# Chang-Tun-Yu/HLS-final-Visual-Odometry

Measured on AMD Instinct MI355X. Metric: stereo frame-pairs/sec (detect+match), KITTI 1241x376; matches bit-exact, higher is better.
Workload: dtype u8; 1 GPU; KITTI 1241x376 stereo quad-match (prev/curr x L/R), default 50x50 bins; noise=0, gpu_max_hw_queues=4, streams_per_gpu=256, frames_in_hbm=8, parallelism=1x independent stream groups

## Files before the change

hls-final-visual-odometry_amd/csrc/kernels_detect.hip:

```cpp
#include "vh_dev.h"
#include <type_traits>

namespace {

__global__ void half_res_kernel(VhImages src, uint8_t *__restrict__ dst, VhGeom g) {
  const int32_t id = blockIdx.z;
  const uint8_t *__restrict__ I = vh_image_ptr(src, id);
  uint8_t *__restrict__ O = dst + (int64_t)id * g.bplm * g.Hm;
  const int32_t u = blockIdx.x * blockDim.x + threadIdx.x;
  const int32_t v = blockIdx.y;
  if (u >= g.bplm) return;
  uint32_t val = 0;
  if (u < g.Wm) {
    const int64_t r0 = (int64_t)(2 * v) * g.bpl + 2 * u, r1 = r0 + g.bpl;
    val = ((uint32_t)I[r0] + I[r0 + 1] + I[r1] + I[r1 + 1]) >> 2;
  }
  O[(int64_t)v * g.bplm + u] = (uint8_t)val;
}

__global__ void __launch_bounds__(256)
detect_nms_kernel(VhImages im, VhGeom g, uint64_t *__restrict__ rec, int32_t *__restrict__ chunk_count) {
  extern __shared__ __attribute__((aligned(16))) uint8_t smem[];
  uint8_t *sI = smem;
  int16_t *sF1 = (int16_t *)(smem + (size_t)g.IH * g.IWp);
  int16_t *sF2 = sF1 + (size_t)g.FH * g.FWp;

  const int32_t id = blockIdx.z;
  const uint8_t *__restrict__ I = vh_image_ptr(im, id);
  const int32_t n = g.n, n1 = n + 1;
  const int32_t bx0 = blockIdx.x * g.tbx, by0 = blockIdx.y * g.tby;
  const int32_t fx0 = VH_MARGIN + bx0 * n1, fy0 = VH_MARGIN + by0 * n1;
  const int32_t ix0 = fx0 - 2, iy0 = fy0 - 2;
  const int32_t tid = threadIdx.x;

  for (int32_t k = tid; k < g.IH * g.IWp; k += 256) {
    const int32_t r = k / g.IWp, c = k - r * g.IWp;
    const int32_t gx = ix0 + c, gy = iy0 + r;
    uint8_t v = 0;
    if (c < g.IW && gx < g.bplm && gy < g.Hm) v = I[(int64_t)gy * g.bplm + gx];
    sI[k] = v;
  }
  __syncthreads();

  {
    const int32_t nseg = max(1, 256 / g.FW);
    const int32_t rows_per = (g.FH + nseg - 1) / nseg;
    for (int32_t task = tid; task < g.FW * nseg; task += 256) {
      const int32_t seg = task / g.FW, cx = task - seg * g.FW;
      const int32_t r0 = seg * rows_per, r1 = min(g.FH, r0 + rows_per);
      if (r0 >= r1) continue;
      int32_t h5[5], h3[5], hc[5], cc[5];
#pragma unroll
      for (int32_t k = 0; k < 4; k++) {
        const uint8_t *p = sI + (size_t)(r0 + k) * g.IWp + cx;
        const int32_t a = p[0], b = p[1], c = p[2], d = p[3], e = p[4];
        h5[k + 1] = a + b + c + d + e; h3[k + 1] = b + c + d; hc[k + 1] = a + b - d - e; cc[k + 1] = c;
      }
      for (int32_t fr = r0; fr < r1; fr++) {
#pragma unroll
        for (int32_t k = 0; k < 4; k++) { h5[k] = h5[k + 1]; h3[k] = h3[k + 1]; hc[k] = hc[k + 1]; cc[k] = cc[k + 1]; }
        const uint8_t *p = sI + (size_t)(fr + 4) * g.IWp + cx;
        const int32_t a = p[0], b = p[1], c = p[2], d = p[3], e = p[4];
        h5[4] = a + b + c + d + e; h3[4] = b + c + d; hc[4] = a + b - d - e; cc[4] = c;
        const int32_t f2 = hc[0] + hc[1] - hc[3] - hc[4];
        const int32_t f1 = -(h5[0] + h5[1] + h5[2] + h5[3] + h5[4]) + 2 * (h3[1] + h3[2] + h3[3]) + 7 * cc[2];
        sF1[(size_t)fr * g.FWp + cx] = (int16_t)f1;
        sF2[(size_t)fr * g.FWp + cx] = (int16_t)f2;
      }
    }
  }
  __syncthreads();

  int32_t *sCnt = (int32_t *)(sF2 + (size_t)g.FH * g.FWp);
  uint32_t *sWork = (uint32_t *)(sCnt + 1);
  uint16_t *sCode = (uint16_t *)(sWork + 4 * g.tbx * g.tby);
  const int32_t nblk_tile = g.tbx * g.tby;
  if (tid == 0) *sCnt = 0;
  for (int32_t k = tid; k < 4 * nblk_tile; k += 256) sCode[k] = VH_NO_CODE;
  __syncthreads();
  const int32_t xlim = (g.Wm - 1 - VH_MARGIN) - fx0, ylim = (g.Hm - 1 - VH_MARGIN) - fy0;
  const int32_t lby = tid / g.tbx, lbx = tid - lby * g.tbx;
  const int32_t bx = bx0 + lbx, by = by0 + lby;
  const bool have_block = tid < nblk_tile && bx < g.nbx && by < g.nby;
  if (have_block) {
    const int32_t fx = n + lbx * n1, fy = n + lby * n1;
    int32_t ex[4], ey[4], ev[4];
    ex[0] = ex[1] = ex[2] = ex[3] = fx;
    ey[0] = ey[1] = ey[2] = ey[3] = fy;
    ev[0] = ev[1] = sF1[(size_t)fy * g.FWp + fx];
    ev[2] = ev[3] = sF2[(size_t)fy * g.FWp + fx];
    for (int32_t j2 = fy; j2 <= fy + n; j2++) {
      for (int32_t i2 = fx; i2 <= fx + n; i2++) {
        int32_t cur = sF1[(size_t)j2 * g.FWp + i2];
        if (cur < ev[0]) { ex[0] = i2; ey[0] = j2; ev[0] = cur; }
        else if (cur > ev[1]) { ex[1] = i2; ey[1] = j2; ev[1] = cur; }
        cur = sF2[(size_t)j2 * g.FWp + i2];
        if (cur < ev[2]) { ex[2] = i2; ey[2] = j2; ev[2] = cur; }
        else if (cur > ev[3]) { ex[3] = i2; ey[3] = j2; ev[3] = cur; }
      }
    }
#pragma unroll
    for (int32_t c = 0; c < 4; c++) {
      const bool pass = (c & 1) ? (ev[c] >= g.tau) : (ev[c] <= -g.tau);
      if (pass) sWork[atomicAdd(sCnt, 1)] = (uint32_t)ex[c] | ((uint32_t)ey[c] << 10) | ((uint32_t)c << 20) | ((uint32_t)tid << 22);
    }
  }
  __syncthreads();
  const int32_t nwork = *sCnt;
  for (int32_t w = tid; w < nwork; w += 256) {
    const uint32_t e = sWork[w];
    const int32_t cx = e & 1023, cy = (e >> 10) & 1023, c = (e >> 20) & 3, owner = e >> 22;
    const int32_t oby = owner / g.tbx, obx = owner - oby * g.tbx;
    const int32_t fx = n + obx * n1, fy = n + oby * n1;
    const int16_t *F = (c < 2) ? sF1 : sF2;
    const bool is_min = (c & 1) == 0;
    const int32_t val = F[(size_t)cy * g.FWp + cx];
    const int32_t jhi = min(cy + n, ylim), ihi = min(cx + n, xlim);
    bool ok = true;
    for (int32_t j2 = cy - n; j2 <= jhi && ok; j2++) {
      for (int32_t i2 = cx - n; i2 <= ihi; i2++) {
        const int32_t cur = F[(size_t)j2 * g.FWp + i2];
        const bool outside = (i2 < fx) | (i2 > fx + n) | (j2 < fy) | (j2 > fy + n);
        if (outside && (is_min ? (cur < val) : (cur > val))) { ok = false; break; }
      }
    }
    if (ok) sCode[owner * 4 + c] = (uint16_t)(((cy - fy) << 6) | (cx - fx));
  }
  __syncthreads();
  if (have_block) {
    uint64_t code = 0;
    int32_t cnt = 0;
#pragma unroll
    for (int32_t c = 0; c < 4; c++) {
      const uint32_t pc = sCode[tid * 4 + c];
      code |= (uint64_t)pc << (16 * c);
      cnt += pc != VH_NO_CODE ? 1 : 0;
    }
    const int32_t blk = by * g.nbx + bx;
    rec[(int64_t)id * g.nblocks + blk] = code;
    if (cnt) atomicAdd(&chunk_count[(int64_t)id * g.nchunks + blk / VH_CHUNK], cnt);
  }
}

#ifdef VH_EMIT_TIMING
__device__ unsigned long long g_emit_t[8];
extern "C" int32_t vh_debug_emit_timing(unsigned long long *out, int32_t reset) {
  if (hipMemcpyFromSymbol(out, HIP_SYMBOL(g_emit_t), sizeof(g_emit_t)) != hipSuccess) return -3;
  if (reset) { unsigned long long z[8] = {0}; z[6] = ~0ull; if (hipMemcpyToSymbol(HIP_SYMBOL(g_emit_t), z, sizeof(z)) != hipSuccess) return -3; }
  return 0;
}
#define VH_TICK_IMPL(k) do { __syncthreads(); if (t_on_) { const unsigned long long now_ = __builtin_readcyclecounter(); atomicAdd(&g_emit_t[k], now_ - t_prev_); t_prev_ = now_; if ((k) == 4) atomicMax(&g_emit_t[7], now_); } } while (0)
#define VH_TICK_INIT_IMPL const bool t_on_ = threadIdx.x == 0 && (blockIdx.x + gridDim.x * (blockIdx.y + gridDim.y * blockIdx.z)) % 61 == 0; unsigned long long t_prev_ = __builtin_readcyclecounter(); if (t_on_) { atomicAdd(&g_emit_t[5], 1ull); atomicMin(&g_emit_t[6], t_prev_); }
#endif
#if defined(VH_EMIT_TIMING) && VH_EMIT_TIMING == 2
#define VH_DTICK(k) VH_TICK_IMPL(k)
#define VH_DTICK_INIT VH_TICK_INIT_IMPL
#else
#define VH_DTICK(k) do { } while (0)
#define VH_DTICK_INIT do { } while (0)
#endif
#if defined(VH_EMIT_TIMING) && VH_EMIT_TIMING != 2
#define VH_ETICK(k) VH_TICK_IMPL(k)
#define VH_ETICK_INIT VH_TICK_INIT_IMPL
#else
#define VH_ETICK(k) do { } while (0)
#define VH_ETICK_INIT do { } while (0)
#endif

template <int N> struct DetTile {
  static constexpr int N1 = N + 1, TBX = 32, TBY = 8;
  static constexpr int FW = TBX * N1 + 2 * N, FH = TBY * N1 + 2 * N;
  static constexpr int IW = FW + 4, IH = FH + 4;
  static constexpr int OFF = (VH_MARGIN - 2) & 3;
  static constexpr int DW = (IW + 3 + 3) / 4;
  static constexpr int IP = DW * 4;
  static constexpr int groups(int px) { return (FW + OFF + px - 1) / px; }
  static constexpr int seg_cost(int px, int s) {
    const int rows = (FH + s - 1) / s, waves = (groups(px) * s + 63) / 64;
    const int hrow = px == 4 ? 28 : 18, vrow = px == 4 ? 26 : 13;
    return groups(px) * s > 256 || rows * (s - 1) >= FH ? (1 << 30) : 1000 * ((rows + 4) * hrow + rows * vrow) + waves;
  }
  static constexpr int best_seg(int px) {
    int b = 1;
    for (int s = 2; s <= 16; s++)
      if (seg_cost(px, s) < seg_cost(px, b)) b = s;
    return b;
  }
#ifdef VH_DET_PX
  static constexpr int PX = VH_DET_PX;
  static constexpr int SEG = VH_DET_SEG;
#else
  static constexpr int PX = seg_cost(2, best_seg(2)) < seg_cost(4, best_seg(4)) ? 2 : 4;
  static constexpr int SEG = best_seg(PX);
#endif
  static constexpr int G = groups(PX);
  static constexpr int FP = PX * G;
  static constexpr int ROWS = (FH + SEG - 1) / SEG;
  static constexpr int BIAS = 8192;
  static_assert((G - 1) * PX / 4 + 1 <= DW - 1, "a group reads the staged dword it starts in and the next one");
  static_assert(G * SEG <= 256, "one lane per (group, row segment)");
  static constexpr int LAST = FH - (SEG - 1) * ROWS;
  static_assert(LAST >= 1, "every segment has rows");
};

template <int N>
__global__ void __launch_bounds__(256)
detect_nms_fast_kernel(VhImages im, VhGeom g, uint64_t *__restrict__ rec, int32_t *__restrict__ chunk_count) {
  using T = DetTile<N>;
  constexpr int N1 = T::N1, WN = 2 * N + 1;
  VH_DET_SETPRIO();
  constexpr int X_BYTES = (T::IH * T::IP > 6144) ? T::IH * T::IP : 6144;
  __shared__ __attribute__((aligned(16))) int16_t sF1[T::FH * T::FP];
  __shared__ __attribute__((aligned(16))) int16_t sF2[T::FH * T::FP];
  __shared__ __attribute__((aligned(16))) uint8_t sX[X_BYTES];
  uint8_t *sI = sX;

  const int32_t id = blockIdx.z, tid = threadIdx.x;
  const uint8_t *__restrict__ I = vh_image_ptr(im, id);
  const int32_t bx0 = blockIdx.x * T::TBX, by0 = blockIdx.y * T::TBY;
  const int32_t fx0 = VH_MARGIN + bx0 * N1, fy0 = VH_MARGIN + by0 * N1;
  const int32_t ix0 = fx0 - 2, iy0 = fy0 - 2;
  const int32_t ax0 = ix0 - T::OFF;
  VH_DTICK_INIT;

  {
    constexpr int NLD = (T::IH * T::DW + 255) / 256;
    uint32_t stg[NLD];
    bool inside[NLD];
#pragma unroll
    for (int32_t i = 0; i < NLD; i++) {
      const int32_t k = min(tid + 256 * i, T::IH * T::DW - 1);
      const int32_t r = k / T::DW, c = k - r * T::DW;
      const int32_t gy = iy0 + r, gx = ax0 + 4 * c;
      stg[i] = *(const uint32_t *)(I + (int64_t)min(gy, g.Hm - 1) * g.bplm + min(gx, g.bplm - 4));
      inside[i] = gy < g.Hm && gx < g.bplm;
    }
    __builtin_amdgcn_sched_barrier(0);
#pragma unroll
    for (int32_t i = 0; i < NLD; i++) {
      const int32_t k = tid + 256 * i;
      if (k < T::IH * T::DW) ((uint32_t *)sI)[k] = inside[i] ? stg[i] : 0u;
    }
  }
  __syncthreads();

  VH_DTICK(0);
  if (tid < T::G * T::SEG) {
    constexpr int PX = T::PX, NR = PX / 2;
    const int32_t seg = tid / T::G, gq = tid - seg * T::G;
    const int32_t r0 = seg * T::ROWS;
    {
      constexpr uint32_t HB = 512u * 0x00010001u, KB = (uint32_t)T::BIAS * 0x00010001u;
      const uint32_t *p = (const uint32_t *)sI + r0 * T::DW + (gq * PX) / 4;
      const uint32_t sel0 = 0x0c010c00u + ((PX == 2 && (gq & 1)) ? 0x00020002u : 0u);
      uint32_t *o1 = (uint32_t *)sF1 + (r0 * T::FP + PX * gq) / 2, *o2 = (uint32_t *)sF2 + (r0 * T::FP + PX * gq) / 2;
      uint32_t h5[NR][5], h3[NR][5], pc[NR][4], cc[NR][5], hcp[NR], S5[NR];
#pragma unroll
      for (int32_t h = 0; h < NR; h++) S5[h] = 0u;
#pragma unroll
      for (int32_t t = 0; t < T::ROWS + 4; t++) {
        if (t - 4 < T::LAST || r0 + t - 4 < T::FH) {
          const uint32_t A = p[t * T::DW], B = p[t * T::DW + 1];
          uint32_t pk[PX + 3];
#pragma unroll
          for (int32_t k = 0; k < PX + 3; k++) pk[k] = __builtin_amdgcn_perm(B, A, sel0 + (uint32_t)k * 0x00010001u);
          uint32_t n5[NR], n3[NR], nc[NR], nz[NR];
          if (PX == 4) {
            const uint32_t a01 = pk[0] + pk[1], a23 = pk[2] + pk[3], a34 = pk[3] + pk[4], a56 = pk[5] + pk[6];
            n3[0] = a23 + pk[1];             n3[NR - 1] = a34 + pk[5];
            n5[0] = n3[0] + pk[0] + pk[4];   n5[NR - 1] = n3[NR - 1] + pk[2] + pk[6];
            nc[0] = (a01 + HB) - a34;        nc[NR - 1] = (a23 + HB) - a56;
            nz[0] = pk[2];                   nz[NR - 1] = pk[4];
          } else {
            n3[0] = pk[1] + pk[2] + pk[3];
            n5[0] = n3[0] + pk[0] + pk[4];
            nc[0] = ((pk[0] + pk[1]) + HB) - (pk[3] + pk[4]);
            nz[0] = pk[2];
          }
          uint32_t f1[NR], f2[NR];
#pragma unroll
          for (int32_t h = 0; h < NR; h++) {
            const uint32_t old5 = h5[h][0];
#pragma unroll
            for (int32_t k = 0; k < 4; k++) { h5[h][k] = h5[h][k + 1]; h3[h][k] = h3[h][k + 1]; cc[h][k] = cc[h][k + 1]; }
            h5[h][4] = n5[h]; h3[h][4] = n3[h]; cc[h][4] = nz[h];
            S5[h] += n5[h];
            if (t >= 5) S5[h] -= old5;
#pragma unroll
            for (int32_t k = 0; k < 3; k++) pc[h][k] = pc[h][k + 1];
            if (t > 0) pc[h][3] = hcp[h] + nc[h];
            hcp[h] = nc[h];
            if (t >= 4) {
              const uint32_t S3 = h3[h][1] + h3[h][2] + h3[h][3];
              f2[h] = (pc[h][0] + KB) - pc[h][3];
              f1[h] = ((S3 + S3) + (__umul24(cc[h][2], 7u) + KB)) - S5[h];
            }
          }
          if (t >= 4) {
            if (PX == 4) {
              *(uint2 *)(o1 + (t - 4) * (T::FP / 2)) = make_uint2(f1[0], f1[NR - 1]);
              *(uint2 *)(o2 + (t - 4) * (T::FP / 2)) = make_uint2(f2[0], f2[NR - 1]);
            } else {
              o1[(t - 4) * (T::FP / 2)] = f1[0];
              o2[(t - 4) * (T::FP / 2)] = f2[0];
            }
          }
        }
      }
    }
  }
  __syncthreads();
  VH_DTICK(1);

  const int32_t xlim = min(max((g.Wm - 1 - VH_MARGIN) - fx0, 0), T::FW - 1);
  const int32_t ylim = min(max((g.Hm - 1 - VH_MARGIN) - fy0, 0), T::FH - 1);
  const int32_t lby = tid / T::TBX, lbx = tid % T::TBX;
  const int32_t bx = bx0 + lbx, by = by0 + lby;
  const bool have_block = bx < g.nbx && by < g.nby;
  const int32_t fx = N + lbx * N1, fy = N + lby * N1;
  constexpr bool PACKED = (N & 1) != 0;
  uint32_t *sQueue = (uint32_t *)sX;
  uint16_t *sCode = (uint16_t *)(sQueue + 1024);
  __shared__ int32_t sQueueN[2];
  if (tid < 2) sQueueN[tid] = 0;
  ((uint2 *)sCode)[tid] = make_uint2(VH_NO_CODE * 0x00010001u, VH_NO_CODE * 0x00010001u);
  __syncthreads();
  {
    typedef int16_t i16x2 __attribute__((ext_vector_type(2)));
    const int32_t lane = tid & 63;
#pragma unroll
    for (int32_t plane = 0; plane < 2; plane++) {
      const int16_t *b = (plane ? sF2 : sF1) + fy * T::FP + fx + T::OFF;
      int32_t vn, vx, pn = 0, px = 0;
      if (PACKED) {
        const i16x2 *bw = (const i16x2 *)b;
        i16x2 mn = bw[0], mx = mn;
#pragma unroll
        for (int32_t j = 0; j < N1; j++) {
#pragma unroll
          for (int32_t d = 0; d < N1 / 2; d++) {
            if (d == 0 && j == 0) continue;
            const i16x2 w = bw[j * (T::FP / 2) + d];
            mn = __builtin_elementwise_min(mn, w);
            mx = __builtin_elementwise_max(mx, w);
          }
        }
        vn = min((int32_t)mn.x, (int32_t)mn.y);
        vx = max((int32_t)mx.x, (int32_t)mx.y);
      } else {
        uint32_t kmin = 0xFFFFFFFFu, kmax = 0u;
#pragma unroll
        for (int32_t j = 0; j < N1; j++) {
#pragma unroll
          for (int32_t i = 0; i < N1; i++) {
            const uint32_t cur = (uint32_t)(uint16_t)b[j * T::FP + i], kk = (uint32_t)((j << 3) | i);
            kmin = min(kmin, (cur << 6) + kk);
            kmax = max(kmax, (cur << 6) + (63u - kk));
          }
        }
        vn = (int32_t)(kmin >> 6); pn = (int32_t)(kmin & 63u);
        vx = (int32_t)(kmax >> 6); px = 63 - (int32_t)(kmax & 63u);
      }
#pragma unroll
      for (int32_t mm = 0; mm < 2; mm++) {
        const bool cand = have_block && (mm ? vx >= T::BIAS + g.tau : vn <= T::BIAS - g.tau);
        const uint32_t payload = PACKED ? (uint32_t)(mm ? vx : vn) : (uint32_t)(mm ? px : pn);
        const uint64_t bal = __ballot(cand);
        if (bal) {
          int32_t base = 0;
          if (lane == 0) base = atomicAdd(&sQueueN[mm], (int32_t)__popcll(bal));
          base = __builtin_amdgcn_readfirstlane(base);
          const int32_t rank = (int32_t)__builtin_amdgcn_mbcnt_hi((uint32_t)(bal >> 32), __builtin_amdgcn_mbcnt_lo((uint32_t)bal, 0u));
          if (cand) sQueue[mm * 512 + base + rank] = (uint32_t)tid | ((uint32_t)(2 * plane + mm) << 8) | (payload << 16);
        }
      }
    }
  }
  __syncthreads();
  VH_DTICK(2);
  {
    const int32_t mm = __builtin_amdgcn_readfirstlane(tid >> 7);
    const int32_t nq = sQueueN[mm];
    const bool unclipped = xlim == T::FW - 1 && ylim == T::FH - 1;
    auto check = [&](auto is_max, auto no_clip) {
      for (int32_t e = tid & 127; e < nq; e += 128) {
        const uint32_t q = sQueue[mm * 512 + e];
        const int32_t owner = q & 255, type = (q >> 8) & 3;
        const int32_t ofy = N + (owner / T::TBX) * N1, ofx = N + (owner % T::TBX) * N1;
        const int16_t *F = ((type & 2) ? sF2 : sF1) + T::OFF;
        int32_t bj = 0, bi = 0;
        if (PACKED) {
          const int32_t val = (int32_t)(q >> 16);
          const int16_t *bb = F + ofy * T::FP + ofx;
#pragma unroll
          for (int32_t idx = N1 * N1 - 1; idx >= 0; idx--) {
            const bool eq = bb[(idx / N1) * T::FP + idx % N1] == val;
            bj = eq ? idx / N1 : bj; bi = eq ? idx % N1 : bi;
          }
        } else {
          bj = (q >> 19) & 7; bi = (q >> 16) & 7;
        }
        const int32_t cy = ofy + bj, cx = ofx + bi;
        int32_t v[WN * WN];
        if (decltype(no_clip)::value) {
          const int16_t *w = F + (cy - N) * T::FP + (cx - N);
#pragma unroll
          for (int32_t j = 0; j < WN; j++)
#pragma unroll
            for (int32_t k = 0; k < WN; k++) v[j * WN + k] = w[j * T::FP + k];
        } else {
          int32_t col[WN];
#pragma unroll
          for (int32_t k = 0; k < WN; k++) col[k] = min(cx - N + k, xlim);
#pragma unroll
          for (int32_t j = 0; j < WN; j++) {
            const int16_t *row = F + min(cy - N + j, ylim) * T::FP;
#pragma unroll
            for (int32_t k = 0; k < WN; k++) v[j * WN + k] = row[col[k]];
          }
        }
        const int32_t centre = v[N * WN + N];
        int32_t ext = centre;
#pragma unroll
        for (int32_t k = 0; k < WN * WN; k++) ext = decltype(is_max)::value ? max(ext, v[k]) : min(ext, v[k]);
        if (ext == centre) sCode[owner * 4 + type] = (uint16_t)((bj << 6) | bi);
      }
    };
    if (mm) { if (unclipped) check(std::true_type{}, std::true_type{}); else check(std::true_type{}, std::false_type{}); }
    else { if (unclipped) check(std::false_type{}, std::true_type{}); else check(std::false_type{}, std::false_type{}); }
  }
  __syncthreads();
  VH_DTICK(3);
  uint32_t codes[4];
  {
    const uint2 cw = ((const uint2 *)sCode)[tid];
    codes[0] = cw.x & 0xFFFFu; codes[1] = cw.x >> 16; codes[2] = cw.y & 0xFFFFu; codes[3] = cw.y >> 16;
  }

  __shared__ int32_t sChunk[16];
  const int32_t chunk_lo = (by0 * g.nbx + bx0) / VH_CHUNK;
  if (tid < 16) sChunk[tid] = 0;
  __syncthreads();
  if (have_block) {
    int32_t cnt = 0;
#pragma unroll
    for (int32_t c = 0; c < 4; c++) cnt += codes[c] != VH_NO_CODE ? 1 : 0;
    const int32_t blk = by * g.nbx + bx;
    rec[(int64_t)id * g.nblocks + blk] = (uint64_t)(codes[0] | (codes[1] << 16)) | ((uint64_t)(codes[2] | (codes[3] << 16)) << 32);
    if (cnt) atomicAdd(&sChunk[blk / VH_CHUNK - chunk_lo], cnt);
  }
  __syncthreads();
  if (tid < 16 && sChunk[tid]) atomicAdd(&chunk_count[(int64_t)id * g.nchunks + chunk_lo + tid], sChunk[tid]);
  VH_DTICK(4);
}

__device__ __forceinline__ int32_t wave_incl_scan(int32_t v) {
#pragma unroll
  for (int32_t d = 1; d < 64; d <<= 1) {
    const int32_t t = __shfl_up(v, d);
    if ((int32_t)(threadIdx.x & 63) >= d) v += t;
  }
  return v;
}

__constant__ int8_t c_desc_dx[16] = {-3, -3, -1, -1, +3, +3, +1, +1, -1, -1, +1, +1, -5, -5, +5, +5};
__constant__ int8_t c_desc_dy[16] = {-1, +1, -1, +1, -1, +1, -1, +1, -5, +5, -5, +5, -3, +3, -3, +3};


#ifndef VH_EMIT_NF
#define VH_EMIT_NF 2
#endif
__global__ void __launch_bounds__(256)
emit_features_kernel(VhImages im, VhGeom g, const uint64_t *__restrict__ rec,
                     const int32_t *__restrict__ chunk_count, VhSets s) {
  int32_t *__restrict__ feat = s.feat;
  int32_t *__restrict__ count = s.count;
  const int32_t cap = s.cap;
  __shared__ uint32_t sList[4 * VH_CHUNK + 1];
  __shared__ int32_t sWave[4], sWaveP[4];

  const int32_t id = blockIdx.y, chunk = blockIdx.x, tid = threadIdx.x;
  const uint8_t *__restrict__ I = vh_image_ptr(im, id);
  const int32_t set = vh_image_set(im, id);
  const int32_t n1 = g.n + 1;
  VH_DET_SETPRIO();
  VH_ETICK_INIT;

  constexpr int BPL = VH_CHUNK / 256;
  uint32_t clo[BPL], chi[BPL];
  {
    const uint2 *rp = reinterpret_cast<const uint2 *>(rec) + (int64_t)id * g.nblocks;
#pragma unroll
    for (int32_t k = 0; k < BPL; k++) {
      const uint2 c = rp[min(chunk * VH_CHUNK + tid * BPL + k, g.nblocks - 1)];
      clo[k] = c.x; chi[k] = c.y;
    }
  }
  int32_t part = 0;
  for (int32_t k = tid; k < chunk; k += 256) part += chunk_count[(int64_t)id * g.nchunks + k];
  int32_t mine = 0;
#pragma unroll
  for (int32_t k = 0; k < BPL; k++) {
    if (chunk * VH_CHUNK + tid * BPL + k >= g.nblocks) clo[k] = chi[k] = ~0u;
    mine += ((clo[k] & 0xFFFFu) != VH_NO_CODE) + ((clo[k] >> 16) != VH_NO_CODE) + ((chi[k] & 0xFFFFu) != VH_NO_CODE) + ((chi[k] >> 16) != VH_NO_CODE);
  }
#pragma unroll
  for (int32_t d = 32; d >= 1; d >>= 1) part += __shfl_xor(part, d);
  const int32_t incl = wave_incl_scan(mine);
  if ((tid & 63) == 63) { sWave[tid >> 6] = incl; sWaveP[tid >> 6] = part; }
  __syncthreads();
  const int32_t base = sWaveP[0] + sWaveP[1] + sWaveP[2] + sWaveP[3];
  VH_ETICK(0);
  int32_t woff = 0;
  for (int32_t w = 0; w < (tid >> 6); w++) woff += sWave[w];
  const int32_t total = sWave[0] + sWave[1] + sWave[2] + sWave[3];
  int32_t pos = woff + incl - mine;
  {
    const int32_t blk0 = chunk * VH_CHUNK + tid * BPL;
    int32_t by = blk0 / g.nbx, bx = blk0 - by * g.nbx;
    const uint32_t org = (uint32_t)(g.n + VH_MARGIN) * ((1u << 14) + 1u);
#pragma unroll
    for (int32_t k = 0; k < BPL; k++) {
      const uint32_t pxy = org + (uint32_t)(bx * n1) + ((uint32_t)(by * n1) << 14);
#pragma unroll
      for (int32_t q = 0; q < 4; q++) {
        const uint32_t w = (q < 2) ? clo[k] : chi[k];
        const uint32_t pc = (q & 1) ? (w >> 16) : (w & 0xFFFFu);
        const bool ok = pc != VH_NO_CODE;
        const uint32_t e = pxy + (pc & 63u) + ((pc >> 6) << 14) + ((uint32_t)q << 28);
        sList[ok ? pos : 4 * VH_CHUNK] = e;
        pos += ok ? 1 : 0;
      }
      if (++bx == g.nbx) { bx = 0; by++; }
    }
  }
  __syncthreads();
  if (chunk == g.nchunks - 1 && tid == 0) count[set] = base + total;
  VH_ETICK(1);
  const int32_t grp = tid >> 4, k = tid & 15;
  const int32_t dx = c_desc_dx[k], dy = c_desc_dy[k];
  constexpr int NF = VH_EMIT_NF;
  const int32_t prk = min(k, 14) - 7;
  typedef uint32_t u32x4a1 __attribute__((ext_vector_type(4), aligned(1)));
  struct Coords { int32_t fs[NF], us[NF], vs[NF], cs[NF]; bool lives[NF]; };
  auto fetch = [&](int32_t f0, Coords &q, u32x4a1 (&prow)[NF]) {
#pragma unroll
    for (int32_t h = 0; h < NF; h++) {
      q.fs[h] = f0 + 16 * h + grp;
      q.lives[h] = q.fs[h] < total;
      const uint32_t e = sList[q.lives[h] ? q.fs[h] : 0];
      q.us[h] = e & 0x3FFF; q.vs[h] = (e >> 14) & 0x3FFF; q.cs[h] = e >> 28;
#ifdef VH_EXP_NOPATCH
      prow[h] = u32x4a1{(uint32_t)q.us[h], (uint32_t)q.vs[h], 0u, 0u};
#else
      prow[h] = *(const u32x4a1 *)(I + (__umul24((uint32_t)(q.vs[h] + prk), (uint32_t)g.bplm) + (uint32_t)(q.us[h] - 7)));
#endif
    }
  };
  Coords qa, qb;
  u32x4a1 pa[NF], pb[NF];
  if (total > 0) fetch(0, qa, pa);

  constexpr int ROWS_LDS = 64;
  __shared__ int32_t sRow[4 * ROWS_LDS];
  __shared__ __attribute__((aligned(16))) uint16_t sLoc[4 * VH_CHUNK];
  const int32_t blk_first = chunk * VH_CHUNK, blk_last = min(blk_first + VH_CHUNK, g.nblocks) - 1;
  const int32_t v_first = ((blk_first / g.nbx) * n1 + g.n + VH_MARGIN) * g.scale;
  const int32_t v_span = ((blk_last / g.nbx) * n1 + g.n + VH_MARGIN + g.n) * g.scale + g.scale - v_first;
  const bool rows_in_lds = v_span <= ROWS_LDS;
  int32_t *__restrict__ rowh = s.row_hist + (int64_t)set * 4 * s.H;
  auto bin_of_entry = [&](uint32_t e) {
    const int32_t uu = (int32_t)(e & 0x3FFF) * g.scale, vv = (int32_t)((e >> 14) & 0x3FFF) * g.scale, c = e >> 28;
    const int32_t ubin = s.binsize == 1 ? uu : (int32_t)__umulhi((uint32_t)uu, s.inv_binsize);
    const int32_t vbin = s.binsize == 1 ? vv : (int32_t)__umulhi((uint32_t)vv, s.inv_binsize);
    return (c * s.ubn + min(ubin, s.ubn - 1)) * s.vbn + min(vbin, s.vbn - 1);
  };
  const bool have0 = tid < total && base + tid < cap;
  const int32_t b0 = have0 ? bin_of_entry(sList[tid]) : 0;
  int32_t slot0 = 0;
  if (have0) slot0 = atomicAdd(&s.hist[(int64_t)set * s.nbins + b0], 1);
  if (rows_in_lds) {
    for (int32_t k = tid; k < 4 * ROWS_LDS; k += 256) sRow[k] = 0;
    __syncthreads();
    for (int32_t f = tid; f < total && base + f < cap; f += 256) {
      const uint32_t e = sList[f];
      const int32_t vv = (int32_t)((e >> 14) & 0x3FFF) * g.scale, c = e >> 28;
      sLoc[f] = (uint16_t)atomicAdd(&sRow[c * ROWS_LDS + (vv - v_first)], 1);
    }
    __syncthreads();
    for (int32_t k = tid; k < 4 * ROWS_LDS; k += 256) {
      const int32_t cnt = sRow[k], c = k / ROWS_LDS, vv = v_first + k % ROWS_LDS;
      if (cnt) sRow[k] = atomicAdd(&rowh[c * s.H + vv], cnt);
    }
    __syncthreads();
  }
  VH_ETICK(2);
  for (int32_t f = tid; f < total; f += 256) {
    const int32_t fi = base + f;
    if (fi >= cap) break;
    const uint32_t e = sList[f];
    const int32_t vv = (int32_t)((e >> 14) & 0x3FFF) * g.scale, c = e >> 28;
    const int32_t b = f == tid ? b0 : bin_of_entry(e);
    const int32_t rowrel = rows_in_lds ? sRow[c * ROWS_LDS + (vv - v_first)] + (int32_t)sLoc[f] : atomicAdd(&rowh[c * s.H + vv], 1);
    const int32_t slot = f == tid ? slot0 : atomicAdd(&s.hist[(int64_t)set * s.nbins + b], 1);
#ifdef VH_CHECK
    { int32_t sl = slot; VH_CHECK_RANGE(s, 5, sl, 0, s.stage_cap); }
#endif
    if (slot < s.stage_cap) s.stage[((int64_t)set * s.nbins + b) * s.stage_cap + slot] = make_int2(fi, rowrel);
  }

  VH_ETICK(3);
  const int32_t sh = g.scale - 1;
  int32_t *__restrict__ out = feat + (int64_t)set * cap * 12;
  uint32_t *__restrict__ fuv = s.f_uv + (int64_t)set * cap;
  const int32_t gbase = (tid & 63) & ~15, j = (k >= 4) ? (k - 4) : 0;
  const uint32_t m_u = k == 0 ? ~0u : 0u, m_v = k == 1 ? ~0u : 0u, m_c = k == 3 ? ~0u : 0u, m_d = k >= 4 ? ~0u : 0u;
  static_assert(16 * NF * 16 * 16 <= (int)sizeof(sLoc), "the patches reuse sLoc");
  __syncthreads();
  uint32_t *sPatch = (uint32_t *)sLoc + grp * (NF * 64);
  const int32_t rd0 = (dy + 5) * 4 + ((dx + 5) >> 2);
  const uint32_t psel = 0x03020100u + (uint32_t)((dx + 5) & 3) * 0x01010101u;
  auto process = [&](const Coords &q, const u32x4a1 (&prow)[NF]) {
    const int32_t *fs = q.fs, *us = q.us, *vs = q.vs, *cs = q.cs;
    const bool *lives = q.lives;
    uint32_t lo[NF][5], hi[NF][5];
    uint32_t sel[NF];
#pragma unroll
    for (int32_t h = 0; h < NF; h++) sel[h] = psel;
    __builtin_amdgcn_sched_barrier(0);
#pragma unroll
    for (int32_t h = 0; h < NF; h++)
      *(uint4 *)(sPatch + (h * 16 + k) * 4) = make_uint4(prow[h].x, prow[h].y, prow[h].z, prow[h].w);
#pragma unroll
    for (int32_t h = 0; h < NF; h++)
#pragma unroll
      for (int32_t r = 0; r < 5; r++) {
        lo[h][r] = sPatch[h * 64 + rd0 + 4 * r];
        hi[h][r] = sPatch[h * 64 + rd0 + 4 * r + 1];
      }
    __builtin_amdgcn_sched_barrier(0);
#pragma unroll
    for (int32_t h = 0; h < NF; h++) {
      const int32_t u = us[h], v = vs[h];
      uint32_t du_p = 0, du_n = 0, dv_p = 0, dv_n = 0;
#pragma unroll
      for (int32_t r = 0; r < 5; r++) {
        const uint32_t w = __builtin_amdgcn_perm(hi[h][r], lo[h][r], sel[h]);
        const uint32_t w1 = __builtin_amdgcn_perm(hi[h][r], lo[h][r], sel[h] + 0x01010101u);
        const uint32_t sw = (r == 0 || r == 4) ? 1u : (r == 2 ? 6u : 4u);
        du_p = __builtin_amdgcn_udot4(w, sw * 0x00000201u, du_p, false);
        du_n = __builtin_amdgcn_udot4(w1, sw * 0x01020000u, du_n, false);
        if (r != 2) {
          const uint32_t dw = (r == 0 || r == 4) ? 1u : 2u;
          uint32_t &acc = r < 2 ? dv_p : dv_n;
          acc = __builtin_amdgcn_udot4(w, dw * 0x00060401u, acc, false);
          acc = __builtin_amdgcn_udot4(w1, dw * 0x01040000u, acc, false);
        }
      }
      const int32_t a_du = (int32_t)(du_p - du_n), a_dv = (int32_t)(dv_p - dv_n);
      const uint32_t du = (uint32_t)min(255, max(0, (a_du >> 7) + 128));
      const uint32_t dv = (uint32_t)min(255, max(0, (a_dv >> 7) + 128));
      const uint32_t pair = du | (dv << 8);
      const uint32_t plo = __shfl(pair, gbase + 2 * j), phi = __shfl(pair, gbase + 2 * j + 1);
      const uint32_t word = (((uint32_t)u << sh) & m_u) | (((uint32_t)v << sh) & m_v) | ((uint32_t)cs[h] & m_c) | ((plo | (phi << 16)) & m_d);
      const int32_t fi = base + fs[h];
      const bool okf = lives[h] && fi < cap;
      if (okf && k < 12) out[(int64_t)fi * 12 + k] = (int32_t)word;
      if (okf && k == 12) fuv[fi] = (uint32_t)(u << sh) | ((uint32_t)(v << sh) << 16);
    }
  };
  if (total > 0) {
    for (int32_t f0 = 0;; f0 += 32 * NF) {
      const bool more1 = f0 + 16 * NF < total;
      if (more1) fetch(f0 + 16 * NF, qb, pb);
      process(qa, pa);
      if (!more1) break;
      const bool more2 = f0 + 32 * NF < total;
      if (more2) fetch(f0 + 32 * NF, qa, pa);
      process(qb, pb);
      if (!more2) break;
    }
  }
  VH_ETICK(4);
}

__global__ void planes_kernel(const uint8_t *__restrict__ I, int32_t bpl, int32_t H,
                              uint8_t *__restrict__ du, uint8_t *__restrict__ dv,
                              int16_t *__restrict__ f1, int16_t *__restrict__ f2) {
  const int32_t x = blockIdx.x * blockDim.x + threadIdx.x, y = blockIdx.y;
  if (x >= bpl) return;
  const int64_t o = (int64_t)y * bpl + x;
  int32_t r_du = 0, r_dv = 0, r_f1 = 0, r_f2 = 0;
  if (x >= 2 && x <= bpl - 3 && y >= 2 && y <= H - 3) {
    int32_t a_du = 0, a_dv = 0, a_f2 = 0, s5 = 0, s3 = 0, ctr = 0;
#pragma unroll
    for (int32_t r = 0; r < 5; r++) {
      const uint8_t *p = I + (int64_t)(y + r - 2) * bpl + (x - 2);
      const int32_t a = p[0], b = p[1], c = p[2], d = p[3], e = p[4];
      const int32_t sw = (r == 0 || r == 4) ? 1 : (r == 2 ? 6 : 4);
      const int32_t dw = (r == 0) ? 1 : (r == 1 ? 2 : (r == 2 ? 0 : (r == 3 ? -2 : -1)));
      const int32_t cw = (r < 2) ? 1 : (r == 2 ? 0 : -1);
      a_du += sw * (a + 2 * b - 2 * d - e);
      a_dv += dw * (a + 4 * b + 6 * c + 4 * d + e);
      a_f2 += cw * (a + b - d - e);
      s5 += a + b + c + d + e;
      if (r >= 1 && r <= 3) s3 += b + c + d;
      if (r == 2) ctr = c;
    }
    r_du = min(255, max(0, (a_du >> 7) + 128));
    r_dv = min(255, max(0, (a_dv >> 7) + 128));
    r_f2 = a_f2;
    if (x >= 3 && y >= 3) r_f1 = -s5 + 2 * s3 + 7 * ctr;
  }
  if (du) du[o] = (uint8_t)r_du;
  if (dv) dv[o] = (uint8_t)r_dv;
  if (f1) f1[o] = (int16_t)r_f1;
  if (f2) f2[o] = (int16_t)r_f2;
}

}

static bool images_dword_aligned(const VhImages &im, const VhGeom &g) {
  return (g.bplm % 4 == 0) && (im.stride % 4 == 0) && ((uintptr_t)im.base[0] % 4 == 0) &&
         (im.ncam < 2 || (uintptr_t)im.base[1] % 4 == 0);
}

void vh_launch_half_res(const VhImages &src, uint8_t *dst, const VhGeom &g, hipStream_t st) {
  dim3 grid((g.bplm + 255) / 256, g.Hm, src.S * src.ncam);
  hipLaunchKernelGGL(half_res_kernel, grid, dim3(256), 0, st, src, dst, g);
}

void vh_launch_detect_nms(const VhImages &im, const VhGeom &g, uint64_t *rec, int32_t *chunk_count,
                          hipStream_t st) {
  if (g.nblocks <= 0) return;
  if (images_dword_aligned(im, g) && g.n >= 1 && g.n <= 4 && g.nbx <= 2048) {
    dim3 grid((g.nbx + 31) / 32, (g.nby + 7) / 8, im.S * im.ncam);
    switch (g.n) {
      case 1: hipLaunchKernelGGL(detect_nms_fast_kernel<1>, grid, dim3(256), 0, st, im, g, rec, chunk_count); break;
      case 2: hipLaunchKernelGGL(detect_nms_fast_kernel<2>, grid, dim3(256), 0, st, im, g, rec, chunk_count); break;
      case 3: hipLaunchKernelGGL(detect_nms_fast_kernel<3>, grid, dim3(256), 0, st, im, g, rec, chunk_count); break;
      default: hipLaunchKernelGGL(detect_nms_fast_kernel<4>, grid, dim3(256), 0, st, im, g, rec, chunk_count); break;
    }
    return;
  }
  dim3 grid((g.nbx + g.tbx - 1) / g.tbx, (g.nby + g.tby - 1) / g.tby, im.S * im.ncam);
  const size_t lds = (size_t)g.IH * g.IWp + 2 * (size_t)g.FH * g.FWp * sizeof(int16_t) + 4 +
                     (size_t)g.tbx * g.tby * (16 + 8);
  hipLaunchKernelGGL(detect_nms_kernel, grid, dim3(256), lds, st, im, g, rec, chunk_count);
}

void vh_launch_emit_features(const VhImages &im, const VhGeom &g, const uint64_t *rec,
                             const int32_t *chunk_count, const VhSets &s, hipStream_t st) {
  if (g.nblocks <= 0) return;
  dim3 grid(g.nchunks, im.S * im.ncam);
  hipLaunchKernelGGL(emit_features_kernel, grid, dim3(256), 0, st, im, g, rec, chunk_count, s);
}

void vh_launch_planes(const uint8_t *img, int32_t bpl, int32_t H, uint8_t *du, uint8_t *dv,
                      int16_t *f1, int16_t *f2, hipStream_t st) {
  dim3 grid((bpl + 255) / 256, H);
  hipLaunchKernelGGL(planes_kernel, grid, dim3(256), 0, st, img, bpl, H, du, dv, f1, f2);
}
```

Measured before the change: 111,000 pairs/s.

## Vectorize tile loads, merge candidate queue atomics, and balance NMS checks across all threads

The image tile load now uses 16-byte vector loads clamped to the image end instead of per-word loads with inside masks, and the tile row pitch is padded to a multiple of 16 bytes. Candidate emission gathers four ballots and issues one packed atomic per wave for both min and max queues. The NMS check loop now spreads the combined min and max queue across all 256 threads, with wave-uniform specialisation and a mixed variant where a wave straddles the two queues. Even N now recovers the argmax position by value search like odd N. Out-of-bounds bytes now come from clamped reads rather than zeros, which relies on those bytes never affecting results, and optional stop-point macros are added for profiling.

```diff
diff --git a/hls-final-visual-odometry_amd/csrc/kernels_detect.hip b/hls-final-visual-odometry_amd/csrc/kernels_detect.hip
--- a/hls-final-visual-odometry_amd/csrc/kernels_detect.hip
+++ b/hls-final-visual-odometry_amd/csrc/kernels_detect.hip
@@ -167,13 +167,25 @@
 #define VH_ETICK_INIT do { } while (0)
 #endif
 
+#ifdef VH_EXP_DET_STOP
+#define VH_DET_STOP(k)                                                                                   \
+  if (VH_EXP_DET_STOP == (k) && g.nbx > 0) {                                                              \
+    const int32_t sbx = bx0 + tid % T::TBX, sby = by0 + tid / T::TBX;                                     \
+    if (sbx < g.nbx && sby < g.nby) rec[(int64_t)id * g.nblocks + sby * g.nbx + sbx] = ~0ull;              \
+    return;                                                                                               \
+  }
+#else
+#define VH_DET_STOP(k) do { } while (0)
+#endif
+
 template <int N> struct DetTile {
   static constexpr int N1 = N + 1, TBX = 32, TBY = 8;
   static constexpr int FW = TBX * N1 + 2 * N, FH = TBY * N1 + 2 * N;
   static constexpr int IW = FW + 4, IH = FH + 4;
   static constexpr int OFF = (VH_MARGIN - 2) & 3;
-  static constexpr int DW = (IW + 3 + 3) / 4;
+  static constexpr int DW = ((IW + 3 + 3) / 4 + 3) / 4 * 4;
   static constexpr int IP = DW * 4;
+  static constexpr int NC = DW / 4;
   static constexpr int groups(int px) { return (FW + OFF + px - 1) / px; }
   static constexpr int seg_cost(int px, int s) {
     const int rows = (FH + s - 1) / s, waves = (groups(px) * s + 63) / 64;
@@ -224,27 +236,28 @@
   VH_DTICK_INIT;
 
   {
-    constexpr int NLD = (T::IH * T::DW + 255) / 256;
-    uint32_t stg[NLD];
-    bool inside[NLD];
+    constexpr int NLD = (T::IH * T::NC + 255) / 256;
+    typedef uint32_t u32x4a4 __attribute__((ext_vector_type(4), aligned(4)));
+    typedef uint32_t u32x4 __attribute__((ext_vector_type(4)));
+    const uint32_t last = (uint32_t)g.Hm * (uint32_t)g.bplm - 16u;
+    u32x4 stg[NLD];
 #pragma unroll
     for (int32_t i = 0; i < NLD; i++) {
-      const int32_t k = min(tid + 256 * i, T::IH * T::DW - 1);
-      const int32_t r = k / T::DW, c = k - r * T::DW;
-      const int32_t gy = iy0 + r, gx = ax0 + 4 * c;
-      stg[i] = *(const uint32_t *)(I + (int64_t)min(gy, g.Hm - 1) * g.bplm + min(gx, g.bplm - 4));
-      inside[i] = gy < g.Hm && gx < g.bplm;
+      const int32_t k = min(tid + 256 * i, T::IH * T::NC - 1);
+      const int32_t r = k / T::NC, c = k - r * T::NC;
+      stg[i] = *(const u32x4a4 *)(I + min((uint32_t)(iy0 + r) * (uint32_t)g.bplm + (uint32_t)(ax0 + 16 * c), last));
     }
     __builtin_amdgcn_sched_barrier(0);
 #pragma unroll
     for (int32_t i = 0; i < NLD; i++) {
       const int32_t k = tid + 256 * i;
-      if (k < T::IH * T::DW) ((uint32_t *)sI)[k] = inside[i] ? stg[i] : 0u;
+      if (k < T::IH * T::NC) ((u32x4 *)sI)[k] = stg[i];
     }
   }
   __syncthreads();
 
   VH_DTICK(0);
+  VH_DET_STOP(1);
   if (tid < T::G * T::SEG) {
     constexpr int PX = T::PX, NR = PX / 2;
     const int32_t seg = tid / T::G, gq = tid - seg * T::G;
@@ -311,6 +324,7 @@
   }
   __syncthreads();
   VH_DTICK(1);
+  VH_DET_STOP(2);
 
   const int32_t xlim = min(max((g.Wm - 1 - VH_MARGIN) - fx0, 0), T::FW - 1);
   const int32_t ylim = min(max((g.Hm - 1 - VH_MARGIN) - fy0, 0), T::FH - 1);
@@ -318,21 +332,22 @@
   const int32_t bx = bx0 + lbx, by = by0 + lby;
   const bool have_block = bx < g.nbx && by < g.nby;
   const int32_t fx = N + lbx * N1, fy = N + lby * N1;
-  constexpr bool PACKED = (N & 1) != 0;
   uint32_t *sQueue = (uint32_t *)sX;
   uint16_t *sCode = (uint16_t *)(sQueue + 1024);
-  __shared__ int32_t sQueueN[2];
-  if (tid < 2) sQueueN[tid] = 0;
+  __shared__ uint32_t sQueueN;
+  if (tid == 0) sQueueN = 0;
   ((uint2 *)sCode)[tid] = make_uint2(VH_NO_CODE * 0x00010001u, VH_NO_CODE * 0x00010001u);
   __syncthreads();
   {
     typedef int16_t i16x2 __attribute__((ext_vector_type(2)));
     const int32_t lane = tid & 63;
+    bool cand[4];
+    uint32_t ext[4];
 #pragma unroll
     for (int32_t plane = 0; plane < 2; plane++) {
       const int16_t *b = (plane ? sF2 : sF1) + fy * T::FP + fx + T::OFF;
-      int32_t vn, vx, pn = 0, px = 0;
-      if (PACKED) {
+      int32_t vn, vx;
+      if (N & 1) {
         const i16x2 *bw = (const i16x2 *)b;
         i16x2 mn = bw[0], mx = mn;
 #pragma unroll
@@ -348,89 +363,97 @@
         vn = min((int32_t)mn.x, (int32_t)mn.y);
         vx = max((int32_t)mx.x, (int32_t)mx.y);
       } else {
-        uint32_t kmin = 0xFFFFFFFFu, kmax = 0u;
-#pragma unroll
-        for (int32_t j = 0; j < N1; j++) {
-#pragma unroll
-          for (int32_t i = 0; i < N1; i++) {
-            const uint32_t cur = (uint32_t)(uint16_t)b[j * T::FP + i], kk = (uint32_t)((j << 3) | i);
-            kmin = min(kmin, (cur << 6) + kk);
-            kmax = max(kmax, (cur << 6) + (63u - kk));
-          }
+        vn = vx = b[0];
+#pragma unroll
+        for (int32_t k = 1; k < N1 * N1; k++) {
+          const int32_t cur = b[(k / N1) * T::FP + k % N1];
+          vn = min(vn, cur);
+          vx = max(vx, cur);
         }
-        vn = (int32_t)(kmin >> 6); pn = (int32_t)(kmin & 63u);
-        vx = (int32_t)(kmax >> 6); px = 63 - (int32_t)(kmax & 63u);
-      }
-#pragma unroll
-      for (int32_t mm = 0; mm < 2; mm++) {
-        const bool cand = have_block && (mm ? vx >= T::BIAS + g.tau : vn <= T::BIAS - g.tau);
-        const uint32_t payload = PACKED ? (uint32_t)(mm ? vx : vn) : (uint32_t)(mm ? px : pn);
-        const uint64_t bal = __ballot(cand);
-        if (bal) {
-          int32_t base = 0;
-          if (lane == 0) base = atomicAdd(&sQueueN[mm], (int32_t)__popcll(bal));
-          base = __builtin_amdgcn_readfirstlane(base);
-          const int32_t rank = (int32_t)__builtin_amdgcn_mbcnt_hi((uint32_t)(bal >> 32), __builtin_amdgcn_mbcnt_lo((uint32_t)bal, 0u));
-          if (cand) sQueue[mm * 512 + base + rank] = (uint32_t)tid | ((uint32_t)(2 * plane + mm) << 8) | (payload << 16);
+      }
+      cand[2 * plane] = have_block && vn <= T::BIAS - g.tau;
+      cand[2 * plane + 1] = have_block && vx >= T::BIAS + g.tau;
+      ext[2 * plane] = (uint32_t)vn;
+      ext[2 * plane + 1] = (uint32_t)vx;
+    }
+    uint64_t bal[4];
+#pragma unroll
+    for (int32_t t = 0; t < 4; t++) bal[t] = __ballot(cand[t]);
+    const uint32_t n0 = (uint32_t)__popcll(bal[0]), n1 = (uint32_t)__popcll(bal[1]);
+    const uint32_t add = (n0 + (uint32_t)__popcll(bal[2])) | ((n1 + (uint32_t)__popcll(bal[3])) << 16);
+    if (add) {
+      uint32_t base = 0;
+      if (lane == 0) base = atomicAdd(&sQueueN, add);
+      base = __builtin_amdgcn_readfirstlane(base);
+#pragma unroll
+      for (int32_t t = 0; t < 4; t++) {
+        const int32_t mm = t & 1;
+        const uint32_t first = ((base >> (16 * mm)) & 0xFFFFu) + (t >= 2 ? (mm ? n1 : n0) : 0u);
+        const uint32_t rank = __builtin_amdgcn_mbcnt_hi((uint32_t)(bal[t] >> 32), __builtin_amdgcn_mbcnt_lo((uint32_t)bal[t], 0u));
+        if (cand[t]) sQueue[mm * 512 + first + rank] = (uint32_t)tid | ((uint32_t)t << 8) | (ext[t] << 16);
+      }
+    }
+  }
+  __syncthreads();
+  VH_DTICK(2);
+  VH_DET_STOP(3);
+  {
+    const int32_t n0 = (int32_t)(sQueueN & 0xFFFFu), ntot = n0 + (int32_t)(sQueueN >> 16);
+    const bool unclipped = xlim == T::FW - 1 && ylim == T::FH - 1;
+    auto check = [&](auto kind, auto no_clip, int32_t e) {
+      const uint32_t q = sQueue[e < n0 ? e : 512 + e - n0];
+      const int32_t owner = q & 255, type = (q >> 8) & 3;
+      const int32_t ofy = N + (owner / T::TBX) * N1, ofx = N + (owner % T::TBX) * N1;
+      const int16_t *F = ((type & 2) ? sF2 : sF1) + T::OFF;
+      const int32_t val = (int32_t)(q >> 16);
+      const int16_t *bb = F + ofy * T::FP + ofx;
+      int32_t pos = (N << 6) | N;
+#pragma unroll
+      for (int32_t idx = N1 * N1 - 2; idx >= 0; idx--)
+        pos = bb[(idx / N1) * T::FP + idx % N1] == val ? (((idx / N1) << 6) | (idx % N1)) : pos;
+      const int32_t bj = pos >> 6, bi = pos & 63;
+      const int32_t cy = ofy + bj, cx = ofx + bi;
+      int32_t v[WN * WN];
+      if (decltype(no_clip)::value) {
+        const int16_t *w = F + (cy - N) * T::FP + (cx - N);
+#pragma unroll
+        for (int32_t j = 0; j < WN; j++)
+#pragma unroll
+          for (int32_t k = 0; k < WN; k++) v[j * WN + k] = w[j * T::FP + k];
+      } else {
+        int32_t col[WN];
+#pragma unroll
+        for (int32_t k = 0; k < WN; k++) col[k] = min(cx - N + k, xlim);
+#pragma unroll
+        for (int32_t j = 0; j < WN; j++) {
+          const int16_t *row = F + min(cy - N + j, ylim) * T::FP;
+#pragma unroll
+          for (int32_t k = 0; k < WN; k++) v[j * WN + k] = row[col[k]];
         }
       }
-    }
-  }
-  __syncthreads();
-  VH_DTICK(2);
-  {
-    const int32_t mm = __builtin_amdgcn_readfirstlane(tid >> 7);
-    const int32_t nq = sQueueN[mm];
-    const bool unclipped = xlim == T::FW - 1 && ylim == T::FH - 1;
-    auto check = [&](auto is_max, auto no_clip) {
-      for (int32_t e = tid & 127; e < nq; e += 128) {
-        const uint32_t q = sQueue[mm * 512 + e];
-        const int32_t owner = q & 255, type = (q >> 8) & 3;
-        const int32_t ofy = N + (owner / T::TBX) * N1, ofx = N + (owner % T::TBX) * N1;
-        const int16_t *F = ((type & 2) ? sF2 : sF1) + T::OFF;
-        int32_t bj = 0, bi = 0;
-        if (PACKED) {
-          const int32_t val = (int32_t)(q >> 16);
-          const int16_t *bb = F + ofy * T::FP + ofx;
-#pragma unroll
-          for (int32_t idx = N1 * N1 - 1; idx >= 0; idx--) {
-            const bool eq = bb[(idx / N1) * T::FP + idx % N1] == val;
-            bj = eq ? idx / N1 : bj; bi = eq ? idx % N1 : bi;
-          }
-        } else {
-          bj = (q >> 19) & 7; bi = (q >> 16) & 7;
-        }
-        const int32_t cy = ofy + bj, cx = ofx + bi;
-        int32_t v[WN * WN];
-        if (decltype(no_clip)::value) {
-          const int16_t *w = F + (cy - N) * T::FP + (cx - N);
-#pragma unroll
-          for (int32_t j = 0; j < WN; j++)
-#pragma unroll
-            for (int32_t k = 0; k < WN; k++) v[j * WN + k] = w[j * T::FP + k];
-        } else {
-          int32_t col[WN];
-#pragma unroll
-          for (int32_t k = 0; k < WN; k++) col[k] = min(cx - N + k, xlim);
-#pragma unroll
-          for (int32_t j = 0; j < WN; j++) {
-            const int16_t *row = F + min(cy - N + j, ylim) * T::FP;
-#pragma unroll
-            for (int32_t k = 0; k < WN; k++) v[j * WN + k] = row[col[k]];
-          }
-        }
-        const int32_t centre = v[N * WN + N];
-        int32_t ext = centre;
-#pragma unroll
-        for (int32_t k = 0; k < WN * WN; k++) ext = decltype(is_max)::value ? max(ext, v[k]) : min(ext, v[k]);
-        if (ext == centre) sCode[owner * 4 + type] = (uint16_t)((bj << 6) | bi);
-      }
+      const int32_t centre = v[N * WN + N];
+      int32_t emin = centre, emax = centre;
+#pragma unroll
+      for (int32_t k = 0; k < WN * WN; k++) {
+        if (decltype(kind)::value != 1) emin = min(emin, v[k]);
+        if (decltype(kind)::value != 0) emax = max(emax, v[k]);
+      }
+      const int32_t ext = decltype(kind)::value == 0 ? emin : decltype(kind)::value == 1 ? emax : ((type & 1) ? emax : emin);
+      if (ext == centre) sCode[owner * 4 + type] = (uint16_t)((bj << 6) | bi);
     };
-    if (mm) { if (unclipped) check(std::true_type{}, std::true_type{}); else check(std::true_type{}, std::false_type{}); }
-    else { if (unclipped) check(std::false_type{}, std::true_type{}); else check(std::false_type{}, std::false_type{}); }
+    typedef std::integral_constant<int, 0> KMin;
+    typedef std::integral_constant<int, 1> KMax;
+    typedef std::integral_constant<int, 2> KBoth;
+    for (int32_t e = tid; e < ntot; e += 256) {
+      const int32_t e0 = __builtin_amdgcn_readfirstlane(e & ~63);
+      if (e0 + 63 < n0) { if (unclipped) check(KMin{}, std::true_type{}, e); else check(KMin{}, std::false_type{}, e); }
+      else if (e0 >= n0) { if (unclipped) check(KMax{}, std::true_type{}, e); else check(KMax{}, std::false_type{}, e); }
+      else { if (unclipped) check(KBoth{}, std::true_type{}, e); else check(KBoth{}, std::false_type{}, e); }
+    }
   }
   __syncthreads();
   VH_DTICK(3);
+  VH_DET_STOP(4);
   uint32_t codes[4];
   {
     const uint2 cw = ((const uint2 *)sCode)[tid];
```

Result: faster. 113,800 pairs/s, median of 6 (+2.5%).
